# Nicolo2277/Vivim

Measured on AMD Instinct MI355X. Metric: frames/sec fwd+bwd, 256x256 clip=5 3-class, higher is better.
Workload: dtype bf16

## Files before the change

### vivim_amd/csrc/wgrad.hip

```cpp
#include "ops.cuh"

namespace vivim {

typedef __attribute__((ext_vector_type(8))) __bf16 wg_bf8;
typedef __attribute__((ext_vector_type(8))) _Float16 wg_h8;
typedef __attribute__((ext_vector_type(4))) float wg_f4;

template <typename T> struct WgFrag;
template <> struct WgFrag<bf16_t> {
    typedef wg_bf8 type;
    static __device__ __forceinline__ wg_f4 mma(type a, type b, wg_f4 c) { return __builtin_amdgcn_mfma_f32_16x16x32_bf16(a, b, c, 0, 0, 0); }
};
template <> struct WgFrag<f16_t> {
    typedef wg_h8 type;
    static __device__ __forceinline__ wg_f4 mma(type a, type b, wg_f4 c) { return __builtin_amdgcn_mfma_f32_16x16x32_f16(a, b, c, 0, 0, 0); }
};

constexpr int kWgMF = 4;


template <typename T, int NF, int DEPTH>
__global__ void __launch_bounds__(kWave) wgrad_nt_kernel(const vivim_wgrad_nt_params p, const int steps_per_split, const int col_tiles) {
    typedef typename WgFrag<T>::type frag;
    const int lane = threadIdx.x, r = lane & 15, kq = lane >> 4;
    const int g = blockIdx.z;
    const int rt = blockIdx.y / col_tiles, ct = blockIdx.y - rt * col_tiles;
    const int m0 = rt * 16 * kWgMF, n0 = ct * 16 * NF;
    const T* __restrict__ a = static_cast<const T*>(p.a) + (int64_t)g * p.a_group_stride;
    const T* __restrict__ b = static_cast<const T*>(p.b) + (int64_t)g * p.b_group_stride;
    const T* arow[kWgMF];
    const T* brow[NF];
#pragma unroll
    for (int i = 0; i < kWgMF; ++i) arow[i] = a + (int64_t)min(m0 + 16 * i + r, p.m - 1) * p.a_row_stride + 8 * kq;
#pragma unroll
    for (int j = 0; j < NF; ++j) brow[j] = b + (int64_t)min(n0 + 16 * j + r, p.n - 1) * p.b_row_stride + 8 * kq;

    wg_f4 acc[kWgMF][NF];
#pragma unroll
    for (int i = 0; i < kWgMF; ++i)
#pragma unroll
        for (int j = 0; j < NF; ++j) acc[i][j] = wg_f4{0.f, 0.f, 0.f, 0.f};

    const int nsteps = (p.k + 31) / 32;
    const int s0 = blockIdx.x * steps_per_split, s1 = min(nsteps, s0 + steps_per_split);
    const frag zero = {};
    auto load = [&](const T* row, int s) -> frag {
        return (s < s1 && 32 * s + 8 * kq < p.k) ? *reinterpret_cast<const frag*>(row + 32 * s) : zero;
    };
    frag fa[DEPTH][kWgMF], fb[DEPTH][NF];
#pragma unroll
    for (int d = 0; d < DEPTH - 1; ++d) {
#pragma unroll
        for (int i = 0; i < kWgMF; ++i) fa[d][i] = load(arow[i], s0 + d);
#pragma unroll
        for (int j = 0; j < NF; ++j) fb[d][j] = load(brow[j], s0 + d);
    }
    for (int s = s0; s < s1; s += DEPTH) {
#pragma unroll
        for (int h = 0; h < DEPTH; ++h) {
            constexpr int D1 = DEPTH - 1;
            const int nxt = (h + D1) % DEPTH;
#pragma unroll
            for (int i = 0; i < kWgMF; ++i) fa[nxt][i] = load(arow[i], s + h + D1);
#pragma unroll
            for (int j = 0; j < NF; ++j) fb[nxt][j] = load(brow[j], s + h + D1);
#pragma unroll
            for (int i = 0; i < kWgMF; ++i)
#pragma unroll
                for (int j = 0; j < NF; ++j) acc[i][j] = WgFrag<T>::mma(fa[h][i], fb[h][j], acc[i][j]);
        }
    }
    float* __restrict__ out = static_cast<float*>(p.out) + (int64_t)g * p.out_group_stride;
#pragma unroll
    for (int i = 0; i < kWgMF; ++i)
#pragma unroll
        for (int j = 0; j < NF; ++j) {
            const int col = n0 + 16 * j + r;
#pragma unroll
            for (int e = 0; e < 4; ++e) {
                const int row = m0 + 16 * i + 4 * kq + e;
                if (row < p.m && col < p.n) atomicAdd(out + (int64_t)row * p.out_row_stride + col, acc[i][j][e]);
            }
        }
}

template <typename T>
static void wgrad_launch(const vivim_wgrad_nt_params& p, hipStream_t stream) {
    const int nf = p.n <= 16 ? 1 : 4;
    const int row_tiles = (p.m + 16 * kWgMF - 1) / (16 * kWgMF), col_tiles = (p.n + 16 * nf - 1) / (16 * nf);
    const int nsteps = (p.k + 31) / 32;
    const int64_t tiles = (int64_t)row_tiles * col_tiles * p.groups;
    const char* ew = getenv("VIVIM_WGRAD_WAVES");
    const char* es = getenv("VIVIM_WGRAD_MINSTEPS");
    const int waves = ew && atoi(ew) > 0 ? atoi(ew) : 2048, minsteps = es && atoi(es) > 0 ? atoi(es) : 16;
    int splits = (int)std::min<int64_t>(std::max<int64_t>(1, waves / tiles), std::max(1, nsteps / minsteps));
    const int sps = (nsteps + splits - 1) / splits;
    splits = (nsteps + sps - 1) / sps;
    const dim3 grid(splits, row_tiles * col_tiles, p.groups), block(kWave);
    if (nf == 1) hipLaunchKernelGGL((wgrad_nt_kernel<T, 1, 4>), grid, block, 0, stream, p, sps, col_tiles);
    else hipLaunchKernelGGL((wgrad_nt_kernel<T, 4, 3>), grid, block, 0, stream, p, sps, col_tiles);
}

bool wgrad_nt_dispatch(const vivim_wgrad_nt_params& p, hipStream_t stream) {
    switch (p.itype) {
        case VIVIM_BF16: wgrad_launch<bf16_t>(p, stream); return true;
        case VIVIM_F16: wgrad_launch<f16_t>(p, stream); return true;
    }
    return false;
}

}
```

### vivim_amd/mamba_simple.py

```python
import math

import torch
import torch.nn as nn
import torch.nn.functional as F

import os

from .dirmap import combine_directions, stack_directions
from .causal_conv1d_interface import causal_conv1d_fn, causal_conv1d_update
from .selective_scan_interface import mamba_inner_fn_no_out_proj, mamba_inner_grouped_fn_no_out_proj, selective_scan_fn
from .selective_state_update import selective_state_update

_DIRECTIONS = ("", "_b", "_s")
_FUSED = ("conv1d{}.weight", "conv1d{}.bias", "x_proj{}.weight", "dt_proj{}.weight", "dt_proj{}.bias", "A{}_log", "D{}")


class _FusedViews(torch.autograd.Function):

    @staticmethod
    def forward(ctx, nb, *args):
        ctx.nb = nb
        return tuple(b.view_as(b) for b in args[:nb])

    @staticmethod
    def backward(ctx, *gs):
        out = [None] * (1 + ctx.nb)
        for g in gs:
            out += [None, None, None] if g is None else [g[0], g[1], g[2]]
        return tuple(out)


class Mamba(nn.Module):
    def __init__(self, d_model, d_state=16, d_conv=4, expand=2, dt_rank="auto", dt_min=0.001, dt_max=0.1,
                 dt_init="random", dt_scale=1.0, dt_init_floor=1e-4, conv_bias=True, bias=False,
                 use_fast_path=True, layer_idx=None, device=None, dtype=None, bimamba_type="none",
                 nframes=5):
        kw = {"device": device, "dtype": dtype}
        super().__init__()
        assert bimamba_type == "v3", "this fork only builds the tri-directional v3 block (mamba_simple.py:125)"
        self.d_model, self.d_state, self.d_conv, self.expand = d_model, d_state, d_conv, expand
        self.d_inner = int(expand * d_model)
        self.dt_rank = math.ceil(d_model / 16) if dt_rank == "auto" else dt_rank
        self.use_fast_path = use_fast_path
        self.layer_idx = layer_idx
        self.bimamba_type = bimamba_type
        self.nframes = nframes
        self.activation = "silu"

        self.in_proj = nn.Linear(d_model, 2 * self.d_inner, bias=bias, **kw)
        for sfx in _DIRECTIONS:
            self.add_module("conv1d" + sfx, nn.Conv1d(self.d_inner, self.d_inner, kernel_size=d_conv,
                                                      groups=self.d_inner, padding=d_conv - 1,
                                                      bias=conv_bias, **kw))
            self.add_module("x_proj" + sfx, nn.Linear(self.d_inner, self.dt_rank + 2 * d_state, bias=False, **kw))
            dt_proj = nn.Linear(self.dt_rank, self.d_inner, bias=True, **kw)
            self.add_module("dt_proj" + sfx, dt_proj)
            if sfx == "":
                std = self.dt_rank ** -0.5 * dt_scale
                if dt_init == "constant":
                    nn.init.constant_(dt_proj.weight, std)
                elif dt_init == "random":
                    nn.init.uniform_(dt_proj.weight, -std, std)
                else:
                    raise NotImplementedError
                dt = torch.exp(torch.rand(self.d_inner, **kw) * (math.log(dt_max) - math.log(dt_min))
                               + math.log(dt_min)).clamp(min=dt_init_floor)
                with torch.no_grad():
                    dt_proj.bias.copy_(dt + torch.log(-torch.expm1(-dt)))
                dt_proj.bias._no_reinit = True
            A_log = torch.log(torch.arange(1, d_state + 1, dtype=torch.float32, device=device)
                              ).repeat(self.d_inner, 1).contiguous()
            a_name = f"A{sfx}_log"
            self.register_parameter(a_name, nn.Parameter(A_log))
            getattr(self, a_name)._no_weight_decay = True
            d_name = "D" + sfx
            self.register_parameter(d_name, nn.Parameter(torch.ones(self.d_inner, device=device)))
            getattr(self, d_name)._no_weight_decay = True
        self.out_proj = nn.Linear(self.d_inner, d_model, bias=bias, **kw)

    def _fuse(self):
        def param(path):
            obj = self
            for name in path.split("."):
                obj = getattr(obj, name)
            return obj
        bufs, groups = [], []
        for kind in _FUSED:
            ps = [param(kind.format(sfx)) for sfx in _DIRECTIONS]
            if any(p is None for p in ps):
                bufs.append(None)
                groups.append(None)
                continue
            buf = torch.stack([p.data for p in ps])
            for g, p in enumerate(ps):
                p.data = buf[g]
            bufs.append(buf)
            groups.append(ps)
        self._fused = bufs
        self._fused_live = [b for b in bufs if b is not None]
        self._fused_args = self._fused_live + [p for ps in groups if ps is not None for p in ps]
        self._fused_where = []
        for kind, buf in zip(_FUSED, bufs):
            if buf is None:
                continue
            for g, sfx in enumerate(_DIRECTIONS):
                *mods, attr = kind.format(sfx).split(".")
                owner = self
                for name in mods:
                    owner = getattr(owner, name)
                self._fused_where.append((owner._parameters, attr, buf[g].data_ptr(), buf.dtype, buf.device))

    def _fused_params(self):
        where = getattr(self, "_fused_where", None)
        ok = where is not None
        if ok:
            args = self._fused_args
            k = len(self._fused_live)
            for i, (params, attr, ptr, dtype, device) in enumerate(where):
                prm = params.get(attr)
                if prm is not args[k + i] or prm.data_ptr() != ptr or prm.dtype != dtype or prm.device != device:
                    ok = False
                    break
        if not ok:
            self._fuse()
        bufs = self._fused
        views = iter(_FusedViews.apply(len(self._fused_live), *self._fused_args))
        return [None if b is None else next(views) for b in bufs]

    def _inner(self, xz, sfx):
        conv, x_proj, dt_proj = (getattr(self, n + sfx) for n in ("conv1d", "x_proj", "dt_proj"))
        A = -torch.exp(getattr(self, f"A{sfx}_log").float())
        return mamba_inner_fn_no_out_proj(
            xz, conv.weight, conv.bias, x_proj.weight, dt_proj.weight, A, None, None,
            getattr(self, "D" + sfx).float(), delta_bias=dt_proj.bias.float(), delta_softplus=True)

    def forward(self, hidden_states, inference_params=None, nframes=None):
        batch, seqlen, _ = hidden_states.shape
        if inference_params is not None:
            conv_state, ssm_state = self._get_states_from_cache(inference_params, batch)
            if inference_params.seqlen_offset > 0:
                return self.step(hidden_states, conv_state, ssm_state)[0]
            return self._prefill(hidden_states, conv_state, ssm_state)
        nf = self.nframes if nframes is None else nframes
        if seqlen % nf != 0:
            raise ValueError(f"seqlen {seqlen} is not a multiple of nframes {nf}")
        xz = (self.in_proj.weight @ hidden_states.reshape(batch * seqlen, -1).t()
              ).view(2 * self.d_inner, batch, seqlen).transpose(0, 1)
        if self.in_proj.bias is not None:
            xz = xz + self.in_proj.bias.to(xz.dtype)[:, None]
        hw = seqlen // nf
        if os.environ.get("VIVIM_SEPARATE_DIRECTIONS", "0") == "1" or seqlen % 8 != 0:
            return self._forward_separate(xz, batch, seqlen, nf, hw)
        D = self.d_inner
        xz3 = stack_directions(xz, nf)
        conv_w, conv_b, x_proj_w, dt_proj_w, dt_bias, A_log, Dp = self._fused_params()
        A = -torch.exp(A_log.float()).view(3 * D, self.d_state)
        o3 = mamba_inner_grouped_fn_no_out_proj(
            xz3, conv_w.view(3 * D, self.d_conv), conv_b.view(3 * D) if conv_b is not None else None, x_proj_w, dt_proj_w,
            A, Dp.float().view(3 * D), dt_bias.float().view(3 * D), True).view(batch, 3, D, seqlen)
        y = combine_directions(o3, nf).transpose(1, 2)
        return F.linear(y, self.out_proj.weight, self.out_proj.bias)

    def _prefill(self, hidden_states, conv_state, ssm_state):
        batch, seqlen, _ = hidden_states.shape
        xz = (self.in_proj.weight @ hidden_states.reshape(batch * seqlen, -1).t()
              ).view(2 * self.d_inner, batch, seqlen).transpose(0, 1)
        if self.in_proj.bias is not None:
            xz = xz + self.in_proj.bias.to(xz.dtype)[:, None]
        x, z = xz.chunk(2, dim=1)
        with torch.no_grad():
            k = min(seqlen, self.d_conv)
            conv_state.zero_()
            conv_state[:, :, self.d_conv - k:].copy_(x[:, :, seqlen - k:])
        x = causal_conv1d_fn(x, self.conv1d.weight.squeeze(1), self.conv1d.bias, self.activation)
        x_dbl = self.x_proj(x.transpose(1, 2).reshape(batch * seqlen, self.d_inner))
        dt, B, C = torch.split(x_dbl, [self.dt_rank, self.d_state, self.d_state], dim=-1)
        dt = (self.dt_proj.weight @ dt.t()).view(self.d_inner, batch, seqlen).transpose(0, 1)
        B = B.reshape(batch, seqlen, self.d_state).transpose(1, 2).contiguous()
        C = C.reshape(batch, seqlen, self.d_state).transpose(1, 2).contiguous()
        y, last_state = selective_scan_fn(x, dt, -torch.exp(self.A_log.float()), B, C, self.D.float(), z=z,
                                          delta_bias=self.dt_proj.bias.float(), delta_softplus=True, return_last_state=True)
        with torch.no_grad():
            ssm_state.copy_(last_state)
        return self.out_proj(y.transpose(1, 2))

    def _get_states_from_cache(self, inference_params, batch_size, initialize_states=False):
        assert self.layer_idx is not None
        if self.layer_idx not in inference_params.key_value_memory_dict:
            inference_params.key_value_memory_dict[self.layer_idx] = self.allocate_inference_cache(batch_size, 0)
        conv_state, ssm_state = inference_params.key_value_memory_dict[self.layer_idx]
        if initialize_states:
            conv_state.zero_()
            ssm_state.zero_()
        return conv_state, ssm_state

    def _forward_separate(self, xz, batch, seqlen, nf, hw):
        out = self._inner(xz, "")
        out_b = self._inner(xz.flip([-1]), "_b").flip([-1])
        xz_s = xz.reshape(batch, 2 * self.d_inner, nf, hw).transpose(2, 3).reshape(batch, 2 * self.d_inner, seqlen)
        out_s = self._inner(xz_s, "_s")
        out_s = out_s.reshape(batch, self.d_inner, hw, nf).transpose(2, 3).reshape(batch, self.d_inner, seqlen)
        y = (out + out_b + out_s).transpose(1, 2) / 3
        return F.linear(y, self.out_proj.weight, self.out_proj.bias)

    def step(self, hidden_states, conv_state, ssm_state):
        assert hidden_states.shape[1] == 1, "Only support decoding with 1 token at a time for now"
        xz = self.in_proj(hidden_states.squeeze(1))
        x, z = xz.chunk(2, dim=-1)
        x = causal_conv1d_update(x.contiguous(), conv_state, self.conv1d.weight.squeeze(1), self.conv1d.bias, self.activation)
        x_db = self.x_proj(x)
        dt, B, C = torch.split(x_db, [self.dt_rank, self.d_state, self.d_state], dim=-1)
        dt = F.linear(dt, self.dt_proj.weight)
        A = -torch.exp(self.A_log.float())
        y = selective_state_update(ssm_state, x, dt, A, B, C, self.D, z=z, dt_bias=self.dt_proj.bias, dt_softplus=True)
        return self.out_proj(y).unsqueeze(1), conv_state, ssm_state

    def allocate_inference_cache(self, batch_size, max_seqlen, dtype=None, **kwargs):
        device = self.out_proj.weight.device
        conv_state = torch.zeros(batch_size, self.d_inner, self.d_conv, device=device,
                                 dtype=self.conv1d.weight.dtype if dtype is None else dtype)
        ssm_state = torch.zeros(batch_size, self.d_inner, self.d_state, device=device,
                                dtype=self.dt_proj.weight.dtype if dtype is None else dtype)
        return conv_state, ssm_state
```

### vivim_amd/optimizer.py

```python
import ctypes

import torch

from . import _lib

SCALE, GROWTH, STEP, NORM, FOUND_INF, FACTOR, BC1, BC2S, SKIPPED, CLIP = range(10)
GROWTH_INTERVAL = 2000


CLASSES = (torch.float32, torch.float16, torch.bfloat16)


def table_order(dtypes):
    return sorted(range(len(dtypes)), key=lambda i: CLASSES.index(dtypes[i]))


def plan(numels, classes=None):
    rows, cuts = [], []
    first = 0
    while first < len(numels):
        count = min(_lib.OPT_MAX_TENSORS, len(numels) - first)
        if classes is not None:
            count = next((k for k in range(1, count) if classes[first + k] != classes[first]), count)
        first_block = len(rows)
# ... 90 lines not shown
            P.masters, P.dtype = base + 24 * n, cls
        return P

    def master_params(self):
        return [p if w is None else w for p, w in zip(self.params, self.masters)]

    def zero_grad(self, set_to_none=True):
        for p in self.params:
            p.grad = None

    def state_dict(self):
        step = self.step_count.to(torch.float32)
        sd = {"lr": self.lr, "betas": self.betas, "eps": self.eps, "weight_decay": self.weight_decay,
              "state": [{"exp_avg": m, "exp_avg_sq": v, "step": step} for m, v in zip(self.exp_avg, self.exp_avg_sq)],
              "record": self.record}
        if self.master_weights:
            sd["master"] = list(self.masters)
        return sd

    def load_state_dict(self, sd):
        assert len(sd["state"]) == len(self.params), "optimizer state does not match the parameter list"
        self.lr, self.betas, self.eps, self.weight_decay = sd["lr"], tuple(sd["betas"]), sd["eps"], sd["weight_decay"]
        with torch.no_grad():
            for m, v, st in zip(self.exp_avg, self.exp_avg_sq, sd["state"]):
                m.copy_(st["exp_avg"])
                v.copy_(st["exp_avg_sq"])
            if sd.get("record") is not None:
                self.record.copy_(sd["record"])
            else:
                steps = torch.stack([torch.as_tensor(st["step"], dtype=torch.float32).to(self.device) for st in sd["state"]])
                self.record[STEP] = steps.max().to(torch.int32)
            saved = sd.get("master") or [None] * len(self.params)
            for p, w, src in zip(self.params, self.masters, saved):
                if w is not None:
                    w.copy_(p.detach().float() if src is None else src)
                    p.copy_(w)

    @torch.no_grad()
    def step(self, max_norm=None, scaled=False):
        if self._addresses() != self._ptrs:
            self._build_tables()
        dev, keep, ptrs = self.device, [], []
        for i in self._live:
            g = self.params[i].grad
            if g is None:
                ptrs.append(None)
                continue
            want = self.params[i].dtype
            if not (g.dtype == want and g.layout == torch.strided and g.device == dev and g.is_contiguous()):
                g = (g if g.layout == torch.strided else g.to_dense()).to(device=dev, dtype=want).contiguous()
                keep.append(g)
            ptrs.append(g.data_ptr())
        if all(q is None for q in ptrs):
            return
        stats = scaled or max_norm is not None
        b1, b2 = self.betas
        for P, grads, _, first, count in self._cuts:
            grads[:] = ptrs[first:first + count]
            P.scaled, P.lr, P.beta1, P.beta2, P.eps, P.weight_decay = int(bool(scaled)), self.lr, b1, b2, self.eps, self.weight_decay
            if stats:
                _lib.launch("vivim_opt_grad_stats" + _suffix(P), P, dev)
        F = self._fin
        F.total_blocks = self.total_blocks if stats else 0
        F.scaled, F.beta1, F.beta2 = int(bool(scaled)), b1, b2
        F.has_max_norm, F.max_norm = (0, 0.0) if max_norm is None else (1, float(max_norm))
        _lib.launch("vivim_opt_finalise", F, dev)
        for P, _, _, _, _ in self._cuts:
            _lib.launch("vivim_opt_adamw" + _suffix(P), P, dev)


def _suffix(P):
    return "_mw" if isinstance(P, _lib.OptMwParams) else ""


_KEEP_FP32 = ("MambaLayer", "_TokenDWConv2d")


def _lowerable(model):
    out, seen = [], set()

    def walk(module):
        if type(module).__name__ in _KEEP_FP32:
            return
        if type(module) in (torch.nn.Linear, torch.nn.Conv2d):
            for p in (module.weight, module.bias):
                if p is not None and id(p) not in seen:
                    seen.add(id(p))
                    out.append(p)
        for child in module.children():
            walk(child)
    walk(model)
    return out


def lower_params(model, dtype):
    if dtype not in (torch.float16, torch.bfloat16):
        raise ValueError("lower_params: dtype must be torch.float16 or torch.bfloat16, got %s" % dtype)
    if getattr(model, "_vivim_param_dtype", None) is not None:
        raise ValueError("lower_params: the model's parameters are already stored in %s; raise_params first" % model._vivim_param_dtype)
    lowered = _lowerable(model)
    for p in lowered:
        if p.dtype != torch.float32:
            raise ValueError("lower_params: expected fp32 parameters, got %s" % p.dtype)
        p.master_fp32 = p.detach().clone()
        p.data = p.data.to(dtype)
    model._vivim_param_dtype = dtype
    return lowered


def raise_params(model, optimizer=None):
    masters = {}
    if optimizer is not None:
        masters = {id(p): w for p, w in zip(optimizer.params, optimizer.masters) if w is not None}
    raised = []
    for p in _lowerable(model):
        w = masters.get(id(p), getattr(p, "master_fp32", None))
        if w is None:
            continue
        p.data = w.detach().clone()
        p.grad = None
        if hasattr(p, "master_fp32"):
            del p.master_fp32
        raised.append(p)
    model._vivim_param_dtype = None
    return raised


def check_autocast_dtype(model, amp_dtype):
    stored = model.__dict__.get("_vivim_param_dtype")
    if stored is not None and stored != amp_dtype:
        raise ValueError("this model's Linear / Conv2d parameters are stored in %s (lower_params): it runs under autocast to that "
                         "dtype only, not %s; raise_params(model, optimizer) restores fp32 parameters" % (stored, amp_dtype))
```

### vivim_amd/train_step.py

```python
import os

import torch
import torch.nn.functional as F

from .optimizer import FusedStepAdamW, check_autocast_dtype, lower_params


def tversky_loss(probs, onehot, alpha=0.3, beta=0.7, smooth=1e-6):
    tp = (probs * onehot).sum(dim=(2, 3))
    fp = (probs * (1 - onehot)).sum(dim=(2, 3))
    fn = ((1 - probs) * onehot).sum(dim=(2, 3))
    tv = (tp + smooth) / (tp + alpha * fp + beta * fn + smooth)
    return (1 - tv.mean(dim=0)).mean()


_ALPHA = {}


def _alpha_tensor(alpha, device, dtype):
    key = (tuple(alpha), str(device), dtype)
    t = _ALPHA.get(key)
    if t is None:
        t = _ALPHA[key] = torch.tensor(alpha, device=device, dtype=dtype)
    return t


def class_balanced_focal_loss(probs, onehot, gamma=2.0, alpha=(0.05, 0.475, 0.475)):
    a = alpha if torch.is_tensor(alpha) else _alpha_tensor(alpha, probs.device, probs.dtype)
    a = a[None, :, None, None]
    weight = onehot * (1 - probs) ** gamma + (1 - onehot) * probs ** gamma
    bce = -onehot * torch.log(probs + 1e-6) - (1 - onehot) * torch.log(1 - probs + 1e-6)
    return (a * weight * bce).mean(dim=(0, 2, 3)).sum()


def recall_focused_loss(logits, targets, num_classes, gamma=2.0, onehot=None, alpha=None):
    probs = F.softmax(logits.float(), dim=1)
    if onehot is None:
        onehot = F.one_hot(targets.long(), num_classes).permute(0, 3, 1, 2).float()
    if alpha is None:
        alpha = (0.05, 0.475, 0.475) if num_classes == 3 else tuple([1.0 / num_classes] * num_classes)
    return 0.4 * class_balanced_focal_loss(probs, onehot, gamma, alpha) + 0.6 * tversky_loss(probs, onehot)


def build_model(num_classes=3, device="cuda", mamba_kwargs=None, drop_path_rate=0.2, fast_backbone_dwconv=True,
                fused_upsample=False, fused_decode_head=False, fast_backbone_layernorm=False, fused_backbone_add_norm=False,
                low_precision_params=None, fused_head_concat=False):
    from .vivim import Vivim, segformer_b3_random
    model = Vivim(in_chans=3, out_chans=num_classes, backbone=segformer_b3_random(),
                  drop_path_rate=drop_path_rate, mamba_kwargs=mamba_kwargs,
                  fast_backbone_dwconv=fast_backbone_dwconv, fused_upsample=fused_upsample,
                  fused_decode_head=fused_decode_head, fast_backbone_layernorm=fast_backbone_layernorm,
                  fused_backbone_add_norm=fused_backbone_add_norm, fused_head_concat=fused_head_concat)
    from .dp import freeze_unused
    freeze_unused(model)
    model = model.to(device)
    if low_precision_params is not None:
        lower_params(model, low_precision_params)
    return model


class LeanFusedAdamW:

    def __init__(self, params, lr=1e-4, betas=(0.9, 0.999), eps=1e-8, weight_decay=1e-2):
        self.params = [p for p in params if p.requires_grad]
        assert self.params and all(p.is_cuda and p.dtype == torch.float32 for p in self.params)
        self.lr, self.betas, self.eps, self.weight_decay = lr, betas, eps, weight_decay
        self.groups = {}
        for p in self.params:
            self.groups.setdefault(p.device, []).append(p)
        self.state = {dev: ([torch.zeros_like(p) for p in ps], [torch.zeros_like(p) for p in ps],
                            [torch.zeros((), dtype=torch.float32, device=dev) for _ in ps])
                      for dev, ps in self.groups.items()}

    def zero_grad(self, set_to_none=True):
        for p in self.params:
            p.grad = None

    def state_dict(self):
        out = {"lr": self.lr, "betas": self.betas, "eps": self.eps, "weight_decay": self.weight_decay, "state": []}
        where = {id(p): (dev, i) for dev, ps in self.groups.items() for i, p in enumerate(ps)}
        for p in self.params:
            dev, i = where[id(p)]
            m, v, t = self.state[dev]
            out["state"].append({"exp_avg": m[i], "exp_avg_sq": v[i], "step": t[i]})
        return out

    def load_state_dict(self, sd):
        assert len(sd["state"]) == len(self.params), "optimizer state does not match the parameter list"
        self.lr, self.betas, self.eps, self.weight_decay = sd["lr"], tuple(sd["betas"]), sd["eps"], sd["weight_decay"]
        where = {id(p): (dev, i) for dev, ps in self.groups.items() for i, p in enumerate(ps)}
        with torch.no_grad():
            for p, st in zip(self.params, sd["state"]):
                dev, i = where[id(p)]
                m, v, t = self.state[dev]
                m[i].copy_(st["exp_avg"]); v[i].copy_(st["exp_avg_sq"]); t[i].copy_(st["step"])

    @torch.no_grad()
    def step(self):
        for dev, ps in self.groups.items():
            exp_avg, exp_avg_sq, steps = self.state[dev]
            grads = [p.grad for p in ps]
            if any(g is None for g in grads):
                keep = [i for i, g in enumerate(grads) if g is not None]
                ps, grads = [ps[i] for i in keep], [grads[i] for i in keep]
                exp_avg, exp_avg_sq, steps = ([exp_avg[i] for i in keep], [exp_avg_sq[i] for i in keep],
                                              [steps[i] for i in keep])
            torch._foreach_add_(steps, 1)
            torch._fused_adamw_(ps, grads, exp_avg, exp_avg_sq, [], steps, lr=self.lr, beta1=self.betas[0],
                                beta2=self.betas[1], weight_decay=self.weight_decay, eps=self.eps, amsgrad=False,
                                maximize=False)


def make_optimizer(model, lr=1e-4, weight_decay=1e-2, capturable=False, fused=None, lean=None, fused_step=False,
                   master_weights=False):
    params = [p for p in model.parameters() if p.requires_grad]
    fused_step = fused_step and not os.environ.get("VIVIM_NO_FUSED_OPTIMIZER")
    if getattr(model, "_vivim_param_dtype", None) is not None and not (fused_step and master_weights):
        raise ValueError("make_optimizer: this model's parameters are stored in %s (lower_params); it needs fused_step=True and "
                         "master_weights=True (and VIVIM_NO_FUSED_OPTIMIZER unset) -- or raise_params(model) to train it in fp32"
                         % model._vivim_param_dtype)
    if fused_step:
        return FusedStepAdamW(params, lr=lr, betas=(0.9, 0.999), weight_decay=weight_decay, master_weights=master_weights)
    on_gpu = bool(params) and all(p.is_cuda and p.dtype == torch.float32 for p in params)
    if fused is None:
        fused = on_gpu and not capturable
    if lean is None:
        lean = fused and on_gpu
    if lean:
        return LeanFusedAdamW(params, lr=lr, betas=(0.9, 0.999), weight_decay=weight_decay)
    kw = {"fused": True} if fused else {"capturable": capturable}
    return torch.optim.AdamW(params, lr=lr, betas=(0.9, 0.999), weight_decay=weight_decay, **kw)


def synthetic_batch(batch, clip_length, image_size, num_classes, device, seed):
    g = torch.Generator(device="cpu").manual_seed(seed)
# ... 93 lines not shown
```

### vivim_amd/vivim.py

```python
import math

import os

import torch
import torch.nn as nn
import torch.nn.functional as F

from . import decode_head as _dh
from . import dwconv as _dw
from . import head_concat as _hc
from . import layernorm as _ln
from . import upsample as _up
from .mamba_simple import Mamba


class DropPath(nn.Module):

    def __init__(self, drop_prob=0.0):
        super().__init__()
        self.drop_prob = drop_prob

    def forward(self, x):
        if self.drop_prob == 0.0 or not self.training:
            return x
        keep = 1.0 - self.drop_prob
        mask = x.new_empty((x.shape[0],) + (1,) * (x.dim() - 1)).bernoulli_(keep).div_(keep)
        return x * mask

    def sample_scale(self, x):
        if self.drop_prob == 0.0 or not self.training:
            return None
        keep = 1.0 - self.drop_prob
        return torch.empty(x.shape[0], dtype=torch.float32, device=x.device).bernoulli_(keep).div_(keep)


def _init_weights(m):
    if isinstance(m, nn.Linear):
        nn.init.trunc_normal_(m.weight, std=0.02)
        if m.bias is not None:
            nn.init.constant_(m.bias, 0)
    elif isinstance(m, nn.LayerNorm):
        nn.init.constant_(m.bias, 0)
        nn.init.constant_(m.weight, 1.0)
    elif isinstance(m, nn.Conv2d):
        fan_out = m.kernel_size[0] * m.kernel_size[1] * m.out_channels // m.groups
        m.weight.data.normal_(0, math.sqrt(2.0 / fan_out))
        if m.bias is not None:
            m.bias.data.zero_()


class LayerNorm(nn.Module):

    def __init__(self, normalized_shape, eps=1e-6, data_format="channels_last"):
        super().__init__()
        if data_format not in ("channels_last", "channels_first"):
            raise NotImplementedError
        self.weight = nn.Parameter(torch.ones(normalized_shape))
        self.bias = nn.Parameter(torch.zeros(normalized_shape))
        self.eps = eps
        self.data_format = data_format
        self.normalized_shape = (normalized_shape,)

    def forward(self, x):
        if self.data_format == "channels_last":
            return F.layer_norm(x, self.normalized_shape, self.weight, self.bias, self.eps)
        mean = x.mean(1, keepdim=True)
        var = (x - mean).pow(2).mean(1, keepdim=True)
        x = (x - mean) / torch.sqrt(var + self.eps)
        return self.weight[:, None, None] * x + self.bias[:, None, None]


class DWConv(nn.Module):

    def __init__(self, dim=768):
        super().__init__()
        self.dwconv = nn.Conv3d(dim, dim, 3, 1, 1, bias=True, groups=dim)

    def forward(self, x, nf, H, W):
        B, _, C = x.shape
        if _dw.supported(x, self.dwconv.weight):
            return _dw.depthwise_conv_tokens(x, self.dwconv.weight, self.dwconv.bias, nf, H, W)
        x = self.dwconv(x.transpose(1, 2).view(B, C, nf, H, W))
        return x.flatten(2).transpose(1, 2)


class Mlp(nn.Module):
    def __init__(self, in_features, hidden_features=None, out_features=None, act_layer=nn.GELU, drop=0.0):
        super().__init__()
        out_features = out_features or in_features
        hidden_features = hidden_features or in_features
        self.fc1 = nn.Linear(in_features, hidden_features)
        self.dwconv = DWConv(hidden_features)
        self.act = act_layer()
        self.fc2 = nn.Linear(hidden_features, out_features)
        self.drop = nn.Dropout(drop)
        self.apply(_init_weights)

    def forward(self, x, nf, H, W):
        x = self.fc1(x)
        conv = self.dwconv.dwconv
        if isinstance(self.act, nn.GELU) and self.act.approximate == "none" and _dw.supported(x, conv.weight) \
                and not os.environ.get("VIVIM_NO_DWCONV_GELU"):
            x = self.drop(_dw.depthwise_conv_gelu_tokens(x, conv.weight, conv.bias, nf, H, W))
        else:
            x = self.drop(self.act(self.dwconv(x, nf, H, W)))
        return self.drop(self.fc2(x))


class MambaLayer(nn.Module):

    def __init__(self, dim, d_state=16, d_conv=4, expand=2, mlp_ratio=4, drop=0.0, drop_path=0.0,
                 act_layer=nn.GELU, fused_add_norm=False):
        super().__init__()
        self.dim = dim
        self.fused_add_norm = fused_add_norm
        self.norm1 = nn.LayerNorm(dim)
        self.mamba = Mamba(d_model=dim, d_state=d_state, d_conv=d_conv, expand=expand, bimamba_type="v3")
        self.drop_path = DropPath(drop_path) if drop_path > 0.0 else nn.Identity()
        self.norm2 = nn.LayerNorm(dim)
        self.mlp = Mlp(in_features=dim, hidden_features=int(dim * mlp_ratio), act_layer=act_layer, drop=drop)
        self.apply(_init_weights)

    @staticmethod
    def _norm(norm, x_flat):
        if (_ln.supported(x_flat, norm.weight) and _ln.worthwhile(x_flat)
                and not os.environ.get("VIVIM_NO_FUSED_LAYERNORM")):
            return _ln.layer_norm_cm(x_flat, norm.weight, norm.bias, norm.eps)
        return norm(x_flat)

    def forward(self, x):
        B, C, nf, H, W = x.shape
        assert C == self.dim
        x_flat = x.reshape(B, C, nf * H * W).transpose(-1, -2)
        branch = self.mamba(self._norm(self.norm1, x_flat), nframes=nf)
        if self.fused_add_norm and self._add_norm_applies(x_flat, branch, self.norm2.weight):
            x_flat, h = _ln.add_layer_norm_cm(x_flat, branch, self.norm2.weight, self.norm2.bias, self.norm2.eps,
                                              self._drop_scale(x_flat))
            branch = self.mlp(h, nf, H, W)
            if self._add_norm_applies(x_flat, branch, None):
                x_flat = _ln.add_cm(x_flat, branch, self._drop_scale(x_flat))
            else:
                x_flat = x_flat + self.drop_path(branch)
            return x_flat.transpose(-1, -2).reshape(B, C, nf, H, W)
        x_flat = x_flat + self.drop_path(branch)
        x_flat = x_flat + self.drop_path(self.mlp(self._norm(self.norm2, x_flat), nf, H, W))
        return x_flat.transpose(-1, -2).reshape(B, C, nf, H, W)

    @staticmethod
    def _add_norm_applies(x_flat, branch, weight):
        return (_ln.add_norm_supported(x_flat, branch, weight) and _ln.worthwhile(x_flat)
                and not os.environ.get("VIVIM_NO_FUSED_LAYERNORM"))

    def _drop_scale(self, x_flat):
        return self.drop_path.sample_scale(x_flat) if isinstance(self.drop_path, DropPath) else None


def _encoder_parts(backbone):
    seg = backbone.segformer
    if hasattr(seg, "encoder"):
        enc = seg.encoder
        return list(enc.patch_embeddings), list(enc.block), list(enc.layer_norm)
    return ([s.patch_embeddings for s in seg.stages], [s.blocks for s in seg.stages],
            [s.layer_norm for s in seg.stages])


class _TokenDWConv2d(nn.Module):

    def __init__(self, hf_module):
        super().__init__()
        self.dwconv = hf_module.dwconv

    def forward(self, hidden_states, height, width):
        if _dw.supported(hidden_states, self.dwconv.weight):
            return _dw.depthwise_conv_tokens(hidden_states, self.dwconv.weight, self.dwconv.bias, 1, height, width)
        b, _, c = hidden_states.shape
        y = self.dwconv(hidden_states.transpose(1, 2).view(b, c, height, width))
        return y.flatten(2).transpose(1, 2)


def _swap_backbone_dwconv(module):
    n = 0
    for m in module.modules():
        inner = getattr(m, "dwconv", None)
        conv = getattr(inner, "dwconv", None)
        if isinstance(conv, nn.Conv2d) and conv.groups == conv.in_channels and conv.kernel_size == (3, 3) \
                and conv.stride == (1, 1) and conv.padding == (1, 1) and not isinstance(inner, _TokenDWConv2d):
            m.dwconv = _TokenDWConv2d(inner)
            n += 1
    return n


def _swap_backbone_droppath(module):
    n = 0
    for m in module.modules():
        dp = getattr(m, "drop_path", None)
        if isinstance(dp, nn.Module) and type(dp).__name__ == "SegformerDropPath":
            m.drop_path = DropPath(float(dp.drop_prob))
            n += 1
    return n


class _BackboneLayerNorm(nn.LayerNorm):
    low_precision_out = False
# ... 36 lines not shown

    def __init__(self, backbone):
        super().__init__()
        pe, blocks, norms = _encoder_parts(backbone)
        self.patch_embeddings = nn.ModuleList(pe)
        self.block = nn.ModuleList(blocks)
        self.layer_norm = nn.ModuleList(norms)


def _run_block(blk, hs, height, width):
    out = blk(hs, height, width)
    return out[0] if isinstance(out, (tuple, list)) else out


def _block_norms(blk):
    for first, second in (("layernorm_before", "layernorm_after"), ("layer_norm_1", "layer_norm_2")):
        n1, n2 = getattr(blk, first, None), getattr(blk, second, None)
        if isinstance(n1, nn.LayerNorm) and isinstance(n2, nn.LayerNorm):
            ok = all(isinstance(getattr(blk, name, None), nn.Module) for name in ("attention", "mlp", "drop_path"))
            return (n1, n2) if ok else None
    return None


def _add_rows(res, branch, drop_path, norm=None):
    if not isinstance(drop_path, (DropPath, nn.Identity)):
        return None
    w = b = None
    if norm is not None:
        w, b = norm.weight, norm.bias
        if w is None or len(norm.normalized_shape) != 1:
            return None
        want = torch.get_autocast_dtype("cuda") if res.is_cuda and torch.is_autocast_enabled("cuda") else res.dtype
        if branch.dtype != want:
            return None
    rows = _ln.tm_add_rows(res, branch, w, b)
    return rows if rows is not None and _ln.tm_add_worthwhile(res) else None


def _add_norm_site(res, branch, drop_path, norm):
    rows = _add_rows(res, branch, drop_path, norm)
    if rows is None:
        h = drop_path(branch) + res
        return h, norm(h)
    scale = drop_path.sample_scale(branch) if isinstance(drop_path, DropPath) else None
    return _ln.add_layer_norm_tm(res, branch, norm.weight, norm.bias, norm.eps, scale=scale, rows=rows)


def _add_site(res, branch, drop_path):
    rows = _add_rows(res, branch, drop_path)
    if rows is None:
        return drop_path(branch) + res
    scale = drop_path.sample_scale(branch) if isinstance(drop_path, DropPath) else None
    return _ln.add_tm(res, branch, scale=scale, rows=rows)


def _run_stage(blocks, hs, height, width):
    pending = None
    for blk in blocks:
        norms = _block_norms(blk)
        if norms is None:
            if pending is not None:
                hs, pending = _add_site(*pending), None
            hs = _run_block(blk, hs, height, width)
            continue
        if pending is None:
            y = norms[0](hs)
        else:
            hs, y = _add_norm_site(*pending, norms[0])
        branch = blk.attention(y, height, width)
        if isinstance(branch, (tuple, list)):
            branch = branch[0]
        dropout = getattr(blk, "hidden_dropout", None)
        if dropout is not None:
            branch = dropout(branch)
        hs, y = _add_norm_site(hs, branch, blk.drop_path, norms[1])
        pending = (hs, blk.mlp(y, height, width), blk.drop_path)
    return hs if pending is None else _add_site(*pending)


class mamba_block(nn.Module):

    def __init__(self, backbone, in_chans=1, depths=[2, 2, 2, 2], dims=[64, 128, 320, 512],
                 drop_path_rate=0.0, layer_scale_init_value=1e-6, out_indices=[0, 1, 2, 3], mamba_kwargs=None,
                 fast_backbone_dwconv=False, fast_backbone_layernorm=False, fused_backbone_add_norm=False):
        super().__init__()
        self.downsample_layers = _Encoder(backbone)
        self.fused_backbone_add_norm = fused_backbone_add_norm
        if fast_backbone_dwconv:
            _swap_backbone_dwconv(self.downsample_layers)
        if fast_backbone_dwconv or fused_backbone_add_norm:
            _swap_backbone_droppath(self.downsample_layers)
        if fast_backbone_layernorm:
            _swap_backbone_layernorm(self.downsample_layers)
        dp_rates = [x.item() for x in torch.linspace(0, drop_path_rate, sum(depths))]
        mk = mamba_kwargs or {}
        self.stages = nn.ModuleList()
        for i in range(len(dims)):
            self.stages.append(nn.Sequential(*[nn.Sequential(MambaLayer(dim=dims[i], drop_path=dp_rates[i], **mk))
                                               for _ in range(depths[i])]))
        self.out_indices = out_indices

    def forward_features(self, x):
        bz, nf = x.shape[:2]
        hs = x.reshape(bz * nf, *x.shape[-3:])
        outs = []
        enc = self.downsample_layers
        for embed, blocks, _norm, mam_stage in zip(enc.patch_embeddings, enc.block, enc.layer_norm, self.stages):
            hs, height, width = embed(hs)
            if self.fused_backbone_add_norm and not os.environ.get("VIVIM_NO_FUSED_LAYERNORM"):
                hs = _run_stage(blocks, hs, height, width)
            else:
                for blk in blocks:
                    hs = _run_block(blk, hs, height, width)
            hs = hs.reshape(bz * nf, height, width, -1).permute(0, 3, 1, 2).contiguous()
            hs = hs.reshape(bz, nf, *hs.shape[-3:]).transpose(1, 2)
            hs = mam_stage(hs)
            hs = hs.transpose(1, 2).reshape(bz * nf, hs.shape[1], height, width)
            outs.append(hs)
        return tuple(outs)

    def forward(self, x):
        return self.forward_features(x)


def segformer_b3_config(num_labels=150):
    from transformers import SegformerConfig
    return SegformerConfig(num_channels=3, num_encoder_blocks=4, depths=[3, 4, 18, 3], sr_ratios=[8, 4, 2, 1],
                           hidden_sizes=[64, 128, 320, 512], patch_sizes=[7, 3, 3, 3], strides=[4, 2, 2, 2],
                           num_attention_heads=[1, 2, 5, 8], mlp_ratios=[4, 4, 4, 4], decoder_hidden_size=768,
                           num_labels=num_labels)


def segformer_b3_random(num_labels=150):
    from transformers import SegformerForSemanticSegmentation
    return SegformerForSemanticSegmentation(segformer_b3_config(num_labels))


class Vivim(nn.Module):

    def __init__(self, in_chans=3, out_chans=3, depths=[2, 2, 2, 2], feat_size=[64, 128, 320, 512],
                 drop_path_rate=0.2, layer_scale_init_value=1e-6, hidden_size: int = 768, norm_name="instance",
                 conv_block: bool = True, res_block: bool = True, spatial_dims=2, with_edge=False,
                 dropout_rate=0.3, backbone=None, mamba_kwargs=None, fast_backbone_dwconv=False,
                 fused_upsample=False, fused_decode_head=False, fast_backbone_layernorm=False,
                 fused_backbone_add_norm=False, fused_head_concat=False) -> None:
        super().__init__()
        self.fused_upsample = fused_upsample
        self.fused_head_concat = fused_head_concat
        self.fused_decode_head = fused_decode_head
        self.hidden_size = hidden_size
        self.in_chans, self.out_chans = in_chans, out_chans
        self.depths, self.feat_size = depths, feat_size
        self.drop_path_rate = drop_path_rate
        self.layer_scale_init_value = layer_scale_init_value
        self.dropout_rate = dropout_rate
        self.spatial_dims = spatial_dims
        if backbone is None:
            from transformers import SegformerForSemanticSegmentation
            backbone = SegformerForSemanticSegmentation.from_pretrained("nvidia/segformer-b3-finetuned-ade-512-512")
        self.encoder = mamba_block(backbone, in_chans, depths=depths, dims=feat_size,
                                   drop_path_rate=drop_path_rate, mamba_kwargs=mamba_kwargs,
                                   fast_backbone_dwconv=fast_backbone_dwconv,
                                   fast_backbone_layernorm=fast_backbone_layernorm,
                                   fused_backbone_add_norm=fused_backbone_add_norm)
        self.decoder = backbone.decode_head
        self.feature_dropout = nn.Dropout2d(dropout_rate)
        self.out = nn.Conv2d(768, out_chans, kernel_size=1)
        self.with_edge = with_edge
        if with_edge:
            self.edgeocr_cls_head = nn.Conv2d(64, 1, kernel_size=1, stride=1, padding=0, bias=True)

    def _upsample(self, x, size):
        if self.fused_upsample:
            return _up.bilinear_upsample(x, size)
        return F.interpolate(x, size=size, mode="bilinear", align_corners=False)

    def _decoder_projections(self):
        dec = self.decoder
        return dec.linear_c if hasattr(dec, "linear_c") else dec.linear_projections

    def decode(self, encoder_hidden_states, bz, nf):
        if (self.fused_decode_head and not os.environ.get("VIVIM_NO_FUSED_HEAD")
                and _dh.applies(self, encoder_hidden_states)):
            return _dh.eval_decode(self, encoder_hidden_states)
        batch_size = encoder_hidden_states[-1].shape[0]
        size0 = encoder_hidden_states[0].shape[2:]
        projections = self._decoder_projections()
        project = lambda state, mlp: mlp(state).permute(0, 2, 1).reshape(batch_size, -1, state.shape[2], state.shape[3])
        states = None
        if self.fused_head_concat and not os.environ.get("VIVIM_NO_HEAD_CONCAT"):
            states = [project(state, mlp) for state, mlp in zip(encoder_hidden_states, projections)]
            if _hc.supported(states[::-1], size0):
                coins = [torch.rand(1).item() > 0.5 for _ in states]
                p = [self.dropout_rate / 2 if coin and self.training else None for coin in coins]
                return self._decode_tail(_hc.upsample_concat(states[::-1], size0, p[::-1]))
        feats = ()
        for i, (state, mlp) in enumerate(zip(encoder_hidden_states, projections)):
            state = states[i] if states is not None else project(state, mlp)
            state = self._upsample(state, size0)
            if torch.rand(1).item() > 0.5:
                state = F.dropout(state, p=self.dropout_rate / 2, training=self.training)
            feats += (state,)
        return self._decode_tail(torch.cat(feats[::-1], dim=1))

    def _decode_tail(self, concat):
        hidden = self.decoder.linear_fuse(concat)
        hidden = self.decoder.activation(self.decoder.batch_norm(hidden))
        hidden = self.decoder.dropout(self.decoder.dropout(hidden))
        hidden = self.feature_dropout(hidden)
        return self.out(hidden)

    def forward(self, x_in):
        bz, nf, nc, h, w = x_in.shape
        outs = self.encoder(x_in)
        logits = self._upsample(self.decode(outs, bz, nf), (h, w))
        if self.with_edge:
            edge = self._upsample(self.edgeocr_cls_head(outs[0]), (h, w))
            return logits, edge
        return logits
```

Before: 250.0.

## Add opt-in split-K wgrad path for linear layers and adaptive tile width

```diff
diff --git a/vivim_amd/csrc/wgrad.hip b/vivim_amd/csrc/wgrad.hip
--- a/vivim_amd/csrc/wgrad.hip
+++ b/vivim_amd/csrc/wgrad.hip
@@ -84,16 +84,38 @@
         }
 }
 
+struct WgKnobs {
+    int waves, minsteps, nf, cus;
+};
+static const WgKnobs& wg_knobs() {
+    static const WgKnobs k = [] {
+        auto num = [](const char* name) {
+            const char* e = getenv(name);
+            return e && atoi(e) > 0 ? atoi(e) : 0;
+        };
+        int dev = 0, cus = 0;
+        if (hipGetDevice(&dev) != hipSuccess || hipDeviceGetAttribute(&cus, hipDeviceAttributeMultiprocessorCount, dev) != hipSuccess || cus <= 0)
+            cus = 256;
+        return WgKnobs{num("VIVIM_WGRAD_WAVES"), num("VIVIM_WGRAD_MINSTEPS"), num("VIVIM_WGRAD_NF"), cus};
+    }();
+    return k;
+}
+
 template <typename T>
 static void wgrad_launch(const vivim_wgrad_nt_params& p, hipStream_t stream) {
-    const int nf = p.n <= 16 ? 1 : 4;
-    const int row_tiles = (p.m + 16 * kWgMF - 1) / (16 * kWgMF), col_tiles = (p.n + 16 * nf - 1) / (16 * nf);
+    const WgKnobs& knobs = wg_knobs();
     const int nsteps = (p.k + 31) / 32;
-    const int64_t tiles = (int64_t)row_tiles * col_tiles * p.groups;
-    const char* ew = getenv("VIVIM_WGRAD_WAVES");
-    const char* es = getenv("VIVIM_WGRAD_MINSTEPS");
-    const int waves = ew && atoi(ew) > 0 ? atoi(ew) : 2048, minsteps = es && atoi(es) > 0 ? atoi(es) : 16;
-    int splits = (int)std::min<int64_t>(std::max<int64_t>(1, waves / tiles), std::max(1, nsteps / minsteps));
+    const int waves = knobs.waves ? knobs.waves : 2048, minsteps = knobs.minsteps ? knobs.minsteps : 16;
+    auto plan = [&](int nf, int* row_tiles, int* col_tiles) {
+        *row_tiles = (p.m + 16 * kWgMF - 1) / (16 * kWgMF), *col_tiles = (p.n + 16 * nf - 1) / (16 * nf);
+        const int64_t tiles = (int64_t)*row_tiles * *col_tiles * p.groups;
+        return (int)std::min<int64_t>(std::max<int64_t>(1, waves / tiles), std::max(1, nsteps / minsteps));
+    };
+    int nf = p.n <= 16 ? 1 : 4, row_tiles, col_tiles;
+    int splits = plan(nf, &row_tiles, &col_tiles);
+    if (nf == 4 && (int64_t)splits * row_tiles * col_tiles * p.groups < knobs.cus) nf = 1;
+    if (knobs.nf == 1 || knobs.nf == 4) nf = knobs.nf;
+    splits = plan(nf, &row_tiles, &col_tiles);
     const int sps = (nsteps + splits - 1) / splits;
     splits = (nsteps + sps - 1) / sps;
     const dim3 grid(splits, row_tiles * col_tiles, p.groups), block(kWave);
diff --git a/vivim_amd/linear_wgrad.py b/vivim_amd/linear_wgrad.py
--- /dev/null
+++ b/vivim_amd/linear_wgrad.py
@@ -0,0 +1,129 @@
+import os
+
+import torch
+import torch.nn.functional as F
+
+from . import _lib
+
+_ITYPE = {torch.float16: _lib.F16, torch.bfloat16: _lib.BF16}
+MIN_TOKENS = 8192
+
+
+def compute_dtype(x):
+    if x.is_cuda and torch.is_autocast_enabled("cuda"):
+        return torch.get_autocast_dtype("cuda")
+    return x.dtype
+
+
+def supported(x, weight, bias=None):
+    if os.environ.get("VIVIM_NO_LINEAR_WGRAD") or not (x.is_cuda and weight.is_cuda and weight.requires_grad):
+        return False
+    if not torch.is_grad_enabled() or _lib.deterministic():
+        return False
+    if weight.dtype != torch.float32 or (bias is not None and bias.dtype != torch.float32) or weight.dim() != 2:
+        return False
+    if x.dim() < 2 or x.shape[-1] != weight.shape[1] or compute_dtype(x) not in _ITYPE or not x.dtype.is_floating_point:
+        return False
+    tokens = x.numel() // x.shape[-1]
+    return tokens >= MIN_TOKENS and tokens % 8 == 0 and tokens > 0
+
+
+def _channel_major(t):
+    C = t.shape[-1]
+    if t.dim() == 3 and t.stride(1) == 1 and t.stride(2) % 8 == 0 and t.data_ptr() % 16 == 0:
+        B, L, _ = t.shape
+        sb, sc = t.stride(0), t.stride(2)
+        if B == 1 or sb == L:
+            return 1, 0, sc, B * L, t
+        if L % 8 == 0 and sb % 8 == 0 and B <= 65535:
+            return B, sb, sc, L, t
+    elif t.dim() == 2 and t.stride(0) == 1 and t.stride(1) % 8 == 0 and t.data_ptr() % 16 == 0:
+        return 1, 0, t.stride(1), t.shape[0], t
+    c = t.reshape(-1, C).t().contiguous()
+    return 1, 0, c.shape[1], c.shape[1], c
+
+
+def _regroup(desc, groups, per_group):
+    g, gs, rs, k, keep = desc
+    if g == groups:
+        return desc
+    return groups, per_group, rs, per_group, keep
+
+
+def _launch(a, da, b, db_, M, N, itype, out):
+    P = _lib.WgradNtParams()
+    P.groups, P.m, P.n, P.k, P.itype = da[0], M, N, da[3], itype
+    P.a_group_stride, P.a_row_stride = da[1], da[2]
+    P.b_group_stride, P.b_row_stride = db_[1], db_[2]
+    P.out_group_stride, P.out_row_stride = 0, N
+    P.a, P.b, P.out = a.data_ptr(), b.data_ptr(), out.data_ptr()
+    _lib.launch("vivim_wgrad_nt", P, out.device)
+
+
+def weight_grad(dy, x, bias=False):
+    M, N = dy.shape[-1], x.shape[-1]
+    da, dx_ = _channel_major(dy), _channel_major(x)
+    db = None
+    if bias:
+        db = da[4].sum(1, dtype=torch.float32) if da[4] is not dy else dy.sum(tuple(range(dy.dim() - 1)), dtype=torch.float32)
+    if da[0] != dx_[0]:
+        groups, per = max(da[0], dx_[0]), min(da[3], dx_[3])
+        da, dx_ = _regroup(da, groups, per), _regroup(dx_, groups, per)
+    out = _lib.zeros(M * N, dy.device).view(M, N)
+    _launch(da[4], da, dx_[4], dx_, M, N, _ITYPE[dy.dtype], out)
+    return (out, db) if bias else out
+
+
+class _WgradFn(torch.autograd.Function):
+
+    @staticmethod
+    def forward(ctx, y, x, weight, bias):
+        ctx.save_for_backward(x)
+        ctx.has_bias = bias is not None
+        return y
+
+    @staticmethod
+    def backward(ctx, dy):
+        x, = ctx.saved_tensors
+        want_db = ctx.has_bias and ctx.needs_input_grad[3]
+        if ctx.needs_input_grad[2]:
+            dw, db = weight_grad(dy, x, bias=True) if want_db else (weight_grad(dy, x), None)
+        else:
+            dw, db = None, (dy.sum(tuple(range(dy.dim() - 1)), dtype=torch.float32) if want_db else None)
+        return dy, None, dw, db
+
+
+def linear(x, weight, bias=None):
+    if not supported(x, weight, bias):
+        return F.linear(x, weight, bias)
+    dt = compute_dtype(x)
+    x16 = x if x.dtype == dt else x.to(dt)
+    w16 = weight.detach().to(dt)
+    b16 = None if bias is None else bias.detach().to(dt)
+    y = F.linear(x16, w16, b16)
+    return _WgradFn.apply(y, x16.detach(), weight, bias)
+
+
+class SplitKLinear(torch.nn.Linear):
+
+    @classmethod
+    def adopt(cls, lin):
+        new = cls.__new__(cls)
+        torch.nn.Module.__init__(new)
+        new.in_features, new.out_features = lin.in_features, lin.out_features
+        new.weight, new.bias = lin.weight, lin.bias
+        new.train(lin.training)
+        return new
+
+    def forward(self, x):
+        return linear(x, self.weight, self.bias)
+
+
+def swap_linears(root):
+    n = 0
+    for m in root.modules():
+        for name, child in list(m.named_children()):
+            if type(child) is torch.nn.Linear:
+                setattr(m, name, SplitKLinear.adopt(child))
+                n += 1
+    return n
diff --git a/vivim_amd/mamba_simple.py b/vivim_amd/mamba_simple.py
--- a/vivim_amd/mamba_simple.py
+++ b/vivim_amd/mamba_simple.py
@@ -6,6 +6,7 @@
 
 import os
 
+from . import linear_wgrad as _lw
 from .dirmap import combine_directions, stack_directions
 from .causal_conv1d_interface import causal_conv1d_fn, causal_conv1d_update
 from .selective_scan_interface import mamba_inner_fn_no_out_proj, mamba_inner_grouped_fn_no_out_proj, selective_scan_fn
@@ -43,6 +44,7 @@
         self.dt_rank = math.ceil(d_model / 16) if dt_rank == "auto" else dt_rank
         self.use_fast_path = use_fast_path
         self.layer_idx = layer_idx
+        self.split_k_linear_wgrad = False
         self.bimamba_type = bimamba_type
         self.nframes = nframes
         self.activation = "silu"
@@ -159,6 +161,11 @@
             xz3, conv_w.view(3 * D, self.d_conv), conv_b.view(3 * D) if conv_b is not None else None, x_proj_w, dt_proj_w,
             A, Dp.float().view(3 * D), dt_bias.float().view(3 * D), True).view(batch, 3, D, seqlen)
         y = combine_directions(o3, nf).transpose(1, 2)
+        return self._out_proj(y)
+
+    def _out_proj(self, y):
+        if self.split_k_linear_wgrad:
+            return _lw.linear(y, self.out_proj.weight, self.out_proj.bias)
         return F.linear(y, self.out_proj.weight, self.out_proj.bias)
 
     def _prefill(self, hidden_states, conv_state, ssm_state):
@@ -201,7 +208,7 @@
         out_s = self._inner(xz_s, "_s")
         out_s = out_s.reshape(batch, self.d_inner, hw, nf).transpose(2, 3).reshape(batch, self.d_inner, seqlen)
         y = (out + out_b + out_s).transpose(1, 2) / 3
-        return F.linear(y, self.out_proj.weight, self.out_proj.bias)
+        return self._out_proj(y)
 
     def step(self, hidden_states, conv_state, ssm_state):
         assert hidden_states.shape[1] == 1, "Only support decoding with 1 token at a time for now"
diff --git a/vivim_amd/optimizer.py b/vivim_amd/optimizer.py
--- a/vivim_amd/optimizer.py
+++ b/vivim_amd/optimizer.py
@@ -196,7 +196,7 @@
     def walk(module):
         if type(module).__name__ in _KEEP_FP32:
             return
-        if type(module) in (torch.nn.Linear, torch.nn.Conv2d):
+        if type(module) in (torch.nn.Linear, torch.nn.Conv2d) or type(module).__name__ == "SplitKLinear":
             for p in (module.weight, module.bias):
                 if p is not None and id(p) not in seen:
                     seen.add(id(p))
diff --git a/vivim_amd/train_step.py b/vivim_amd/train_step.py
--- a/vivim_amd/train_step.py
+++ b/vivim_amd/train_step.py
@@ -43,6 +43,7 @@
 
 
 def build_model(num_classes=3, device="cuda", mamba_kwargs=None, drop_path_rate=0.2, fast_backbone_dwconv=True,
+                split_k_linear_wgrad=False,
                 fused_upsample=False, fused_decode_head=False, fast_backbone_layernorm=False, fused_backbone_add_norm=False,
                 low_precision_params=None, fused_head_concat=False):
     from .vivim import Vivim, segformer_b3_random
@@ -50,7 +51,8 @@
                   drop_path_rate=drop_path_rate, mamba_kwargs=mamba_kwargs,
                   fast_backbone_dwconv=fast_backbone_dwconv, fused_upsample=fused_upsample,
                   fused_decode_head=fused_decode_head, fast_backbone_layernorm=fast_backbone_layernorm,
-                  fused_backbone_add_norm=fused_backbone_add_norm, fused_head_concat=fused_head_concat)
+                  fused_backbone_add_norm=fused_backbone_add_norm, fused_head_concat=fused_head_concat,
+                  split_k_linear_wgrad=split_k_linear_wgrad and low_precision_params is None)
     from .dp import freeze_unused
     freeze_unused(model)
     model = model.to(device)
diff --git a/vivim_amd/vivim.py b/vivim_amd/vivim.py
--- a/vivim_amd/vivim.py
+++ b/vivim_amd/vivim.py
@@ -10,6 +10,7 @@
 from . import dwconv as _dw
 from . import head_concat as _hc
 from . import layernorm as _ln
+from . import linear_wgrad as _lw
 from . import upsample as _up
 from .mamba_simple import Mamba
 
@@ -85,8 +86,10 @@
 
 
 class Mlp(nn.Module):
-    def __init__(self, in_features, hidden_features=None, out_features=None, act_layer=nn.GELU, drop=0.0):
-        super().__init__()
+    def __init__(self, in_features, hidden_features=None, out_features=None, act_layer=nn.GELU, drop=0.0,
+                 split_k_linear_wgrad=False):
+        super().__init__()
+        self.split_k_linear_wgrad = split_k_linear_wgrad
         out_features = out_features or in_features
         hidden_features = hidden_features or in_features
         self.fc1 = nn.Linear(in_features, hidden_features)
@@ -96,29 +99,34 @@
         self.drop = nn.Dropout(drop)
         self.apply(_init_weights)
 
+    def _linear(self, fc, x):
+        return _lw.linear(x, fc.weight, fc.bias) if self.split_k_linear_wgrad else fc(x)
+
     def forward(self, x, nf, H, W):
-        x = self.fc1(x)
+        x = self._linear(self.fc1, x)
         conv = self.dwconv.dwconv
         if isinstance(self.act, nn.GELU) and self.act.approximate == "none" and _dw.supported(x, conv.weight) \
                 and not os.environ.get("VIVIM_NO_DWCONV_GELU"):
             x = self.drop(_dw.depthwise_conv_gelu_tokens(x, conv.weight, conv.bias, nf, H, W))
         else:
             x = self.drop(self.act(self.dwconv(x, nf, H, W)))
-        return self.drop(self.fc2(x))
+        return self.drop(self._linear(self.fc2, x))
 
 
 class MambaLayer(nn.Module):
 
     def __init__(self, dim, d_state=16, d_conv=4, expand=2, mlp_ratio=4, drop=0.0, drop_path=0.0,
-                 act_layer=nn.GELU, fused_add_norm=False):
+                 act_layer=nn.GELU, fused_add_norm=False, split_k_linear_wgrad=False):
         super().__init__()
         self.dim = dim
         self.fused_add_norm = fused_add_norm
         self.norm1 = nn.LayerNorm(dim)
         self.mamba = Mamba(d_model=dim, d_state=d_state, d_conv=d_conv, expand=expand, bimamba_type="v3")
+        self.mamba.split_k_linear_wgrad = split_k_linear_wgrad
         self.drop_path = DropPath(drop_path) if drop_path > 0.0 else nn.Identity()
         self.norm2 = nn.LayerNorm(dim)
-        self.mlp = Mlp(in_features=dim, hidden_features=int(dim * mlp_ratio), act_layer=act_layer, drop=drop)
+        self.mlp = Mlp(in_features=dim, hidden_features=int(dim * mlp_ratio), act_layer=act_layer, drop=drop,
+                       split_k_linear_wgrad=split_k_linear_wgrad)
         self.apply(_init_weights)
 
     @staticmethod
@@ -321,7 +329,8 @@
 
     def __init__(self, backbone, in_chans=1, depths=[2, 2, 2, 2], dims=[64, 128, 320, 512],
                  drop_path_rate=0.0, layer_scale_init_value=1e-6, out_indices=[0, 1, 2, 3], mamba_kwargs=None,
-                 fast_backbone_dwconv=False, fast_backbone_layernorm=False, fused_backbone_add_norm=False):
+                 fast_backbone_dwconv=False, fast_backbone_layernorm=False, fused_backbone_add_norm=False,
+                 split_k_linear_wgrad=False):
         super().__init__()
         self.downsample_layers = _Encoder(backbone)
         self.fused_backbone_add_norm = fused_backbone_add_norm
@@ -331,11 +340,14 @@
             _swap_backbone_droppath(self.downsample_layers)
         if fast_backbone_layernorm:
             _swap_backbone_layernorm(self.downsample_layers)
+        if split_k_linear_wgrad:
+            _lw.swap_linears(self.downsample_layers.block)
         dp_rates = [x.item() for x in torch.linspace(0, drop_path_rate, sum(depths))]
         mk = mamba_kwargs or {}
         self.stages = nn.ModuleList()
         for i in range(len(dims)):
-            self.stages.append(nn.Sequential(*[nn.Sequential(MambaLayer(dim=dims[i], drop_path=dp_rates[i], **mk))
+            self.stages.append(nn.Sequential(*[nn.Sequential(MambaLayer(dim=dims[i], drop_path=dp_rates[i],
+                                                                      split_k_linear_wgrad=split_k_linear_wgrad, **mk))
                                                for _ in range(depths[i])]))
         self.out_indices = out_indices
 
@@ -380,7 +392,7 @@
     def __init__(self, in_chans=3, out_chans=3, depths=[2, 2, 2, 2], feat_size=[64, 128, 320, 512],
                  drop_path_rate=0.2, layer_scale_init_value=1e-6, hidden_size: int = 768, norm_name="instance",
                  conv_block: bool = True, res_block: bool = True, spatial_dims=2, with_edge=False,
-                 dropout_rate=0.3, backbone=None, mamba_kwargs=None, fast_backbone_dwconv=False,
+                 dropout_rate=0.3, backbone=None, mamba_kwargs=None, fast_backbone_dwconv=False, split_k_linear_wgrad=False,
                  fused_upsample=False, fused_decode_head=False, fast_backbone_layernorm=False,
                  fused_backbone_add_norm=False, fused_head_concat=False) -> None:
         super().__init__()
@@ -401,7 +413,8 @@
                                    drop_path_rate=drop_path_rate, mamba_kwargs=mamba_kwargs,
                                    fast_backbone_dwconv=fast_backbone_dwconv,
                                    fast_backbone_layernorm=fast_backbone_layernorm,
-                                   fused_backbone_add_norm=fused_backbone_add_norm)
+                                   fused_backbone_add_norm=fused_backbone_add_norm,
+                                   split_k_linear_wgrad=split_k_linear_wgrad)
         self.decoder = backbone.decode_head
         self.feature_dropout = nn.Dropout2d(dropout_rate)
         self.out = nn.Conv2d(768, out_chans, kernel_size=1)
```

Result: slower. 209.2 (-16.3%).
